# FrontierDevelopmentLab/2024-HL-SPI3S-SuNeRF

Hardware: AMD Instinct MI355X
Metric: ray-samples/sec (fwd+bwd, fused emission renderer) (higher is better)
Workload: dtype f32 (forward: every operand split into an fp16 head and an exact remainder, head products on the fp16 matrix cores + block-scaled fp8 products for the two cross terms; backward: fp16 MFMA, W^T as a single fp16 image (measured policy); fp32 accumulate and parameters)

## Files before the change

2024-hl-spi3s-sunerf_amd/csrc/bwd_pipe.hip:

```cpp
#include "grad_common.h"
#include <mutex>
#include <vector>

namespace {

constexpr int PD = 256, PKS = PD / 16, PNT = PD / 32, PT = 8;
constexpr int WG = 512;
constexpr int WG_PRE = 256;
constexpr int NBUF = 4;
constexpr int NBUF_H = 5;
#ifndef PIPE_DMA_ON_WEIGHT
#define PIPE_DMA_ON_WEIGHT 2
#endif
#ifndef PIPE_ZD
#define PIPE_ZD 2
#endif
#ifndef PIPE_RING
#define PIPE_RING 16
#endif
#ifndef PIPE_POLL_LAG
#define PIPE_POLL_LAG 2
#endif
constexpr int RING = PIPE_RING;
constexpr int SLOT = PKS * 1024;
constexpr int BUF_HID = 24 * 1024;
constexpr int BUF_IN = 16 * 1024;
constexpr int BUF_PRE = 19 * 1024;
constexpr unsigned SPIN_LIMIT = 50000000u;

constexpr unsigned ST_OK = 0, ST_START_TIMEOUT = 1, ST_PLACEMENT = 2, ST_WAIT_TIMEOUT = 3;

struct PipeArgs {
  const char* packedT;
  const char* act_stash;
  const char* dz_top;
  char* rings;
  unsigned* ctrl;
  float* partial;
  const float* g_raw;
  const unsigned* g_absmax_bits;
  float* partial_out;
  int64_t n_chunks_total;
  int S, n_chunks;
  int n_linear, d_out;
  int NP, NPX;
  int hi_only;
  int inject;
  unsigned* dbg;
};

__host__ __device__ inline size_t ctrl_counter_word(int n_links, int P, int link, int which) {
  return 64 + (((size_t)P * n_links + link) * 4 + which) * 32;
}
__host__ __device__ inline size_t ctrl_bytes(int NP, int n_links) { return (64 + (size_t)NP * n_links * 4 * 32) * 4; }

typedef __attribute__((address_space(1))) unsigned gu32;
__device__ __forceinline__ unsigned ld_agent(const unsigned* p) {
  return __hip_atomic_load((const gu32*)p, __ATOMIC_RELAXED, __HIP_MEMORY_SCOPE_AGENT);
}
__device__ __forceinline__ void st_agent(unsigned* p, unsigned v) {
  __hip_atomic_store((gu32*)p, v, __ATOMIC_RELAXED, __HIP_MEMORY_SCOPE_AGENT);
}

template <int POLICY>
__device__ __forceinline__ void dma_piece(const char* src_lane, unsigned lds_dst) {
  const unsigned d = __builtin_amdgcn_readfirstlane(lds_dst);
  if (POLICY == 1) asm volatile("s_mov_b32 m0, %1\n\ts_nop 0\n\tglobal_load_lds_dwordx4 %0, off nt" :: "v"(src_lane), "s"(d) : "memory");
  else if (POLICY == 2) asm volatile("s_mov_b32 m0, %1\n\ts_nop 0\n\tglobal_load_lds_dwordx4 %0, off sc1" :: "v"(src_lane), "s"(d) : "memory");
  else asm volatile("s_mov_b32 m0, %1\n\ts_nop 0\n\tglobal_load_lds_dwordx4 %0, off" :: "v"(src_lane), "s"(d) : "memory");
}
template <int POLICY>
__device__ __forceinline__ void dma_piece_s(const char* src_uniform, unsigned voff, unsigned lds_dst) {
  const unsigned d = __builtin_amdgcn_readfirstlane(lds_dst);
#ifndef PIPE_STREAM_BITS
#define PIPE_STREAM_BITS "nt"
#endif
  if (POLICY == 1) asm volatile("s_mov_b32 m0, %1\n\ts_nop 0\n\tglobal_load_lds_dwordx4 %0, %2 " PIPE_STREAM_BITS :: "v"(voff), "s"(d), "s"(src_uniform) : "memory");
  else if (POLICY == 2) asm volatile("s_mov_b32 m0, %1\n\ts_nop 0\n\tglobal_load_lds_dwordx4 %0, %2 sc1" :: "v"(voff), "s"(d), "s"(src_uniform) : "memory");
  else asm volatile("s_mov_b32 m0, %1\n\ts_nop 0\n\tglobal_load_lds_dwordx4 %0, %2" :: "v"(voff), "s"(d), "s"(src_uniform) : "memory");
}
__device__ __forceinline__ void dma_poll(const unsigned* src_lane, unsigned lds_dst) {
  const unsigned d = __builtin_amdgcn_readfirstlane(lds_dst);
  asm volatile("s_mov_b32 m0, %1\n\ts_nop 0\n\tglobal_load_lds_dword %0, off sc1" :: "v"(src_lane), "s"(d) : "memory");
}

__device__ __forceinline__ void store_tile(const f32x16& t, float* dst) {
  const Rsrc r = make_rsrc(dst, 16 * 64 * 4);
  const int lo4 = (int)(threadIdx.x & 63u) * 4;
#pragma unroll
  for (int g = 0; g < 16; ++g) {
    const float te = t[g];
    unsigned tv;
    asm volatile("v_accvgpr_read_b32 %0, %1" : "=v"(tv) : "a"(te));
    __builtin_amdgcn_raw_buffer_store_b32(tv, r, lo4, g * 256, 0);
    if ((g & 3) == 3) __builtin_amdgcn_sched_barrier(0);
  }
}

__device__ __forceinline__ void mfma_agpr(f32x16& acc, const half8& a, const half8& b) {
  asm volatile("v_mfma_f32_32x32x16_f16 %0, %1, %2, %0" : "+a"(acc) : "v"(a), "v"(b));
}
__device__ __forceinline__ void drain_matrix_pipe() { asm volatile("s_nop 15\n\ts_nop 15\n\ts_nop 15\n\ts_nop 15" ::: "memory"); }

#ifndef PIPE_KO_WREADS
#define PIPE_KO_WREADS 0
#endif
#if PIPE_KO_WREADS
#define TR_FIXED(R0, R1, R2, R3, OFF, var, base) asm volatile("" : "={v[" #R0 ":" #R3 "]}"(var) : "v"(base) : "memory")
#else
#define TR_FIXED(R0, R1, R2, R3, OFF, var, base)                                                                        \
  asm volatile("ds_read_b64_tr_b16 v[" #R0 ":" #R1 "], %1 offset:%2\n\tds_read_b64_tr_b16 v[" #R2 ":" #R3 "], %1 offset:%3" \
// ... 112 lines not shown
  const char* srcP0 = a.act_stash + SL.h_off(l - 1) + (size_t)(8 * j) * 1024;
  const int64_t safe = cbeg < a.n_chunks_total ? cbeg : a.n_chunks_total - 1;

  constexpr int ZD = TOP ? NBUF_H - 1 : PIPE_ZD;
  const char *nz = nullptr, *np = nullptr;
  unsigned zdst = 0, pdst = 0;
  bool zreal = false, preal = false;
  const char* const safe_p = srcP0 + (size_t)safe * act_chunk;
  const char* const safe_z = TOP ? a.dz_top + (size_t)safe * SLOT : ring_in;
  const char* run_p = srcP0 + (size_t)cbeg * act_chunk;
  const char* run_z = TOP ? a.dz_top + (size_t)cbeg * SLOT : ring_in;
  int run_slot = 0, run_zbuf = 0, run_pbuf = 0;
  auto next_p = [&](int nxt) __attribute__((always_inline)) {
    preal = nxt < n_my;
    pdst = lds0 + run_pbuf * BUF_HID + 16 * 1024;
    run_pbuf = run_pbuf + 1 == NBUF_H ? 0 : run_pbuf + 1;
    np = preal ? run_p : safe_p;
    run_p += act_chunk;
  };
  auto next_z = [&](int nxt) __attribute__((always_inline)) {
    if (nxt < 0) { zreal = false; nz = safe_z; return; }
    zreal = nxt < n_my;
    zdst = lds0 + run_zbuf * BUF_HID;
    run_zbuf = run_zbuf + 1 == NBUF_H ? 0 : run_zbuf + 1;
    nz = zreal ? run_z : safe_z;
    if (TOP) run_z += SLOT;
    else {
      run_slot = run_slot + 1 == RING ? 0 : run_slot + 1;
      run_z = run_slot == 0 ? ring_in : run_z + SLOT;
    }
  };
  auto piece_z = [&](int f) __attribute__((always_inline)) {
    const unsigned dst = zreal ? zdst + f * 1024 : lds_dummy;
    if (TOP) dma_piece_s<1>(nz + (size_t)f * 1024, voff, dst);
    else dma_piece_s<2>(nz + (size_t)f * 1024, voff, dst);
  };
  auto piece_p = [&](int f) __attribute__((always_inline)) { dma_piece_s<1>(np + (size_t)f * 1024, voff, preal ? pdst + f * 1024 : lds_dummy); };
  constexpr int NO = 2;
  constexpr int NP_D = PIPE_DMA_ON_WEIGHT == 0 ? 6 : PIPE_DMA_ON_WEIGHT == 1 ? 4 : 0;
  constexpr int NP_W = 6 - NP_D;
  constexpr int PER_D = NP_D + NO;
  auto min3 = [](int x, int y, int z) constexpr { return x < y ? (x < z ? x : z) : (y < z ? y : z); };
  constexpr int WAIT_LEFT = NP_D == 0 ? NO : min3((ZD - 1) * PER_D + (NP_D - 4) + NO, NP_D == 6 ? 2 * PER_D + NO : 63, 2 * PER_D);
  constexpr int DRAIN = (WAIT_LEFT + PER_D - 1) / PER_D + 1;
  auto w_wait = [min3](int per_w, bool gate_wave) constexpr {
    return min3(NP_W == 6 ? (ZD - 1) * per_w + 2 : 63, NP_W >= 2 ? 2 * per_w : 63, gate_wave ? PIPE_POLL_LAG * per_w - 2 : 63);
  };
  constexpr int W_WAIT_GATE = w_wait(NP_W + 2, true), W_WAIT_REST = w_wait(NP_W, false);

  static_assert(W_WAIT_GATE >= 0 && W_WAIT_GATE < 64 && WAIT_LEFT < 64, "vmcnt is a 6-bit counter");
  static_assert(ZD >= 1 && ZD <= NBUF_H - 1, "dZ fetch distance");

  if (wave < 4) {
#if defined(PIPE_PRIO) && PIPE_PRIO == 1
    __builtin_amdgcn_s_setprio(1);
#endif
#ifndef PIPE_PF
#define PIPE_PF 4
#endif
    constexpr int PF = PIPE_PF;
    const int U = 4 * j + wave;
    const int li = (a.n_linear - 2) - l;
    half8 wt_hi[PKS], wt_lo[HI_ONLY ? 1 : PKS];
    {
      const char* blk = a.packedT + (size_t)PNT * 1024 + ((size_t)li * PNT + U) * PKS * 2048 + lane * 16;
#pragma unroll
      for (int s = 0; s < PKS; ++s) {
        wt_hi[s] = *(const half8*)(blk + s * 2048);
        if constexpr (!HI_ONLY) wt_lo[s] = *(const half8*)(blk + s * 2048 + 1024);
      }
#pragma unroll
      for (int s = 0; s < PKS; ++s) {
        asm volatile("" : "+a"(wt_hi[s]));
        if constexpr (!HI_ONLY) asm volatile("" : "+a"(wt_lo[s]));
      }
    }
    char* scratch = a.rings + (size_t)a.NP * n_links * RING * SLOT + ((size_t)blockIdx.x * 4 + wave) * 2048;
    float cosn[16];
    v2f cosn2[8];
    typedef __attribute__((address_space(3))) v4u lds_v4u;
    typedef __attribute__((address_space(3))) half8 lds_half8;
    v4u dp[2];
    auto read_phases = [&](int b) __attribute__((always_inline)) {
      const unsigned at = lds0 + b * BUF_HID + (16 + 2 * wave) * 1024 + voff;
// ... 109 lines not shown
    if (PIPE_TRIM) {
#pragma unroll
      for (int q = 0; q < 8; ++q) { bs[2 * q] = bs2[q].x; bs[2 * q + 1] = bs2[q].y; }
    }
    store_bias_sums(bs, a.partial + ((size_t)(l - 1) * a.NP + P) * (PT * (PT + 1)) * 1024 + ((size_t)U * (PT + 1) + PT) * 1024);
    if (stamp && P == 0 && lane == 0) {
      unsigned long long* t = (unsigned long long*)(a.dbg + 256 * 8 * 4) + (((size_t)(blockIdx.x >> 3) * 8 + wave) * 8);
      for (int k = 0; k < 5; ++k) t[k] = tl[k];
    }
    if (stamp && wave == 1 && lane == 0) {
      unsigned* d = a.dbg + 256 * 8 + (size_t)blockIdx.x * 8;
      for (int k = 0; k < 6; ++k) d[k] = (unsigned)(ph[k] >> 4);
    }
    return;
  }

#if defined(PIPE_PRIO) && PIPE_PRIO == 2
  __builtin_amdgcn_s_setprio(1);
#endif
  const int v = wave - 4;
  const bool gatew = v == 0;
  const int rq = v >> 1, cq = v & 1;
  const int r0 = 4 * rq, c0 = 2 * cq;
  f32x16 acc[4][2];
  {
    half8 hz = {0, 0, 0, 0, 0, 0, 0, 0};
    asm volatile("s_nop 7" : "+v"(hz));
#pragma unroll
    for (int i = 0; i < 4; ++i) {
      asm volatile("v_mfma_f32_32x32x16_f16 %0, %1, %1, 0" : "=a"(acc[i][0]) : "v"(hz));
      asm volatile("v_mfma_f32_32x32x16_f16 %0, %1, %1, 0" : "=a"(acc[i][1]) : "v"(hz));
    }
  }
  unsigned* in_prod0 = a.ctrl + ctrl_counter_word(n_links, P, TOP ? 0 : l, 0);
  unsigned* in_prod1 = a.ctrl + ctrl_counter_word(n_links, P, TOP ? 0 : l, 1);
  unsigned* my_cons = a.ctrl + ctrl_counter_word(n_links, P, TOP ? 0 : l, 2 + j);
  unsigned* my_prod = a.ctrl + ctrl_counter_word(n_links, P, l - 1, j);
  unsigned* out_cons0 = a.ctrl + ctrl_counter_word(n_links, P, l - 1, 2 + (l == 1 ? j : 0));
  unsigned* out_cons1 = a.ctrl + ctrl_counter_word(n_links, P, l - 1, 2 + (l == 1 ? j : 1));
  const unsigned* poll_src = (lane & 3) == 0 ? in_prod0 : (lane & 3) == 1 ? in_prod1 : (lane & 3) == 2 ? out_cons0 : out_cons1;
  unsigned have_in = 0, have_out = 0;
  unsigned st_in[2] = {0, 0}, st_out[2] = {0, 0};
  const unsigned long long t_begin = __builtin_amdgcn_s_memrealtime();
  const unsigned laneoff = tr_lane_offset(lane);

  auto gate = [&](int itn) __attribute__((always_inline)) {
    const int nx = itn + ZD;
    const bool need_in = !TOP && nx >= 0 && nx < n_my && (int)(have_in - (unsigned)(nx + 1)) < 0;
    const bool need_out = itn >= RING && (int)(have_out - (unsigned)(itn - RING + 1)) < 0;
    if (need_in || need_out) {
      bool ok = true;
      if (lane == 0) {
        if (need_in) ok = spin_until(in_prod0, in_prod1, (unsigned)(nx + 1), status, have_in, st_in);
        if (ok && need_out) ok = spin_until(out_cons0, out_cons1, (unsigned)(itn - RING + 1), status, have_out, st_out);
        if (!ok) lds_st(lds_abort + (itn & 1) * 4, 1u);
      }
      have_in = __builtin_amdgcn_readfirstlane(have_in);
      have_out = __builtin_amdgcn_readfirstlane(have_out);
    }
  };
  if (gatew) {
    if (lane == 0) { lds_st(lds_abort, 0u); lds_st(lds_abort + 4, 0u); }
    gate(-(NBUF_H - 1));
  }

  bool aborted = false;
  unsigned long long tw = 0, tb = 0;
  unsigned long long t_wait = 0, t_bar = 0, tl[6] = {0, 0, 0, 0, 0, 0};
  const bool stamp = a.dbg != nullptr;
  int pslot = PIPE_POLL_LAG;
  auto top = [&](int it) __attribute__((always_inline)) {
    unsigned long long sa = 0, sb = 0;
    if (stamp) sa = __builtin_amdgcn_s_memtime();
    if (gatew) asm volatile("s_waitcnt vmcnt(%0)" :: "i"(W_WAIT_GATE) : "memory");
    else if (NP_W) asm volatile("s_waitcnt vmcnt(%0)" :: "i"(W_WAIT_REST) : "memory");
    if (stamp) sb = __builtin_amdgcn_s_memtime();
    barrier_mem();
    if (stamp) { t_wait = sb; t_bar = __builtin_amdgcn_s_memtime(); tw += sb - sa; tb += t_bar - sb; }
    const unsigned ab = lds_ld(lds_abort + (it & 1) * 4);
    if (gatew) {
      if (lane < 2) {
// ... 74 lines not shown
      ph[0] += s1 - s0; ph[1] += s2 - s1; ph[2] += s3 - s2;
      if (it == n_my / 2) { tl[0] = s0; tl[1] = t_wait; tl[2] = t_bar; tl[3] = s1; tl[4] = s2; tl[5] = s3; }
    }
    if (ab) { aborted = true; break; }
  }
  drain_matrix_pipe();
  if (stamp && (v == 0 || v == 1) && lane == 0) {
    unsigned* d = a.dbg + 256 * 8 * (2 + v) + (size_t)blockIdx.x * 8;
    for (int k = 0; k < 3; ++k) d[k] = (unsigned)(ph[k] >> 4);
    d[3] = (unsigned)(tw >> 4); d[4] = (unsigned)(tb >> 4);
  }
  if (stamp && P == 0 && lane == 0) {
    unsigned long long* t = (unsigned long long*)(a.dbg + 256 * 8 * 4) + (((size_t)(blockIdx.x >> 3) * 8 + wave) * 8);
    for (int k = 0; k < 6; ++k) t[k] = tl[k];
  }
  asm volatile("s_waitcnt vmcnt(0)" ::: "memory");
  barrier_mem();
  if (!aborted && gatew && lane < 2) st_agent(lane == 0 ? my_cons : my_prod, (unsigned)n_my);
  if (a.dbg && gatew && lane == 0) {
    unsigned* d = a.dbg + (size_t)blockIdx.x * 8;
    d[0] = (unsigned)(__builtin_amdgcn_s_memrealtime() - t_begin); d[1] = st_in[0]; d[2] = st_in[1]; d[3] = st_out[0]; d[4] = st_out[1];
    d[5] = (unsigned)n_my; d[6] = (unsigned)l; d[7] = (unsigned)P;
  }

  float* out = a.partial + ((size_t)l * a.NP + P) * (PT * (PT + 1)) * 1024;
#pragma unroll
  for (int i = 0; i < 4; ++i)
#pragma unroll
    for (int jj = 0; jj < 2; ++jj) {
      store_tile(acc[i][jj], out + ((size_t)(r0 + i) * (PT + 1) + (4 * j + c0 + jj)) * 1024);
    }
}

__device__ __forceinline__ void in_stage(const PipeArgs& a, char* smem, int P, int j, int64_t cbeg, int n_my) {
  constexpr int PW = 4;
  const int tid = threadIdx.x, lane = tid & 63;
  const int wave = __builtin_amdgcn_readfirstlane(tid >> 6);
  if (wave >= 4) {
    for (int it = -(NBUF - 1); it < n_my; ++it) {
      barrier_mem();
      if (lds_ld((unsigned)(uintptr_t)smem + NBUF * BUF_IN + 1024 + NBUF * 256 + (it & 1) * 4)) break;
    }
    barrier_mem();
    return;
  }
  const int n_act = a.n_linear - 1, n_links = n_act - 1;
  const StashLayout SL(PD, a.n_linear, true);
  const unsigned lds0 = (unsigned)(uintptr_t)smem;
  const unsigned lds_dummy = lds0 + NBUF * BUF_IN;
  const unsigned lds_poll = lds_dummy + 1024;
  const unsigned lds_abort = lds_poll + NBUF * 256;
  unsigned* status = a.ctrl;

  f32x16 acc[3];
#pragma unroll
  for (int c = 0; c < 3; ++c) acc[c] = (f32x16){0};

  const char* ring_in = a.rings + ((size_t)P * n_links + 0) * RING * SLOT;
  unsigned* in_prod = a.ctrl + ctrl_counter_word(n_links, P, 0, j);
  unsigned* my_cons = a.ctrl + ctrl_counter_word(n_links, P, 0, 2 + j);
  unsigned have_in = 0;
  unsigned st_in[2] = {0, 0};
  const unsigned long long t_begin = __builtin_amdgcn_s_memrealtime();
  const size_t act_chunk = SL.chunk_bytes();
  const unsigned laneoff = tr_lane_offset(lane);
  const int64_t safe = cbeg < a.n_chunks_total ? cbeg : a.n_chunks_total - 1;

  auto issue_chunk = [&](int c, int buf) __attribute__((always_inline)) {
    const bool real = c < n_my;
    const int64_t g = real ? cbeg + c : safe;
    const unsigned dst0 = lds0 + buf * BUF_IN;
    const char* z = ring_in + (size_t)((real ? c : 0) % RING) * SLOT + (size_t)(8 * j) * 1024 + lane * 16;
    const char* e = a.act_stash + (size_t)g * act_chunk + lane * 16;
#pragma unroll
    for (int k = 0; k < PW; ++k) {
      const int p = 4 * k + wave;
      if (k < 2) dma_piece<2>(z + (size_t)p * 1024, real ? dst0 + p * 1024 : lds_dummy);
      else {
        const bool use = real && p < 14;
        dma_piece<1>(e + (size_t)(p < 14 ? p - 8 : 0) * 1024, use ? dst0 + p * 1024 : lds_dummy);
      }
    }
  };

  bool aborted = false;
  for (int it = -(NBUF - 1); it < n_my; ++it) {
    const int buf = it & (NBUF - 1);
    const int nxt = it + NBUF - 1;
    if (wave == 0) asm volatile("s_waitcnt vmcnt(%0)" :: "i"(2 * (PW + 2)) : "memory");
    else asm volatile("s_waitcnt vmcnt(%0)" :: "i"(2 * PW) : "memory");
    if (wave == 0) {
      bool ok = true;
      if (it >= 0) {
        const unsigned p0 = lds_ld(lds_poll + buf * 256);
        if ((int)(p0 - have_in) > 0) have_in = p0;
      }
      if (lane == 0) {
        if (nxt < n_my && (int)(have_in - (unsigned)(nxt + 1)) < 0) ok = spin_until(in_prod, in_prod, (unsigned)(nxt + 1), status, have_in, st_in);
        lds_st(lds_abort + (it & 1) * 4, ok ? 0u : 1u);
      }
      have_in = __builtin_amdgcn_readfirstlane(have_in);
    }
    barrier_mem();
    if (lds_ld(lds_abort + (it & 1) * 4)) { aborted = true; break; }
    if (wave == 0) {
      if (lane == 0) st_agent(my_cons, (unsigned)(it + 1 > 0 ? it + 1 : 0));
      dma_poll(in_prod, lds_poll + (nxt & (NBUF - 1)) * 256);
    }
    issue_chunk(nxt, nxt & (NBUF - 1));
    if (it < 0) continue;
#if defined(PIPE_ABL_IN_STAGE) && PIPE_ABL_IN_STAGE
    continue;
#endif
    const unsigned bufA = lds0 + buf * BUF_IN + laneoff, bufB = bufA + 8 * 1024;
#pragma unroll
    for (int ks = 0; ks < 2; ++ks) {
      half4 alo, ahi, blo[3], bhi[3];
// ... 44 lines not shown
    const unsigned old = __hip_atomic_fetch_or((gu32*)(a.ctrl + 8 + x), mine, __ATOMIC_RELAXED, __HIP_MEMORY_SCOPE_AGENT);
    asm volatile("s_waitcnt vmcnt(0)" ::: "memory");
    (void)old;
    __hip_atomic_fetch_add((gu32*)(a.ctrl + 1), 1u, __ATOMIC_RELAXED, __HIP_MEMORY_SCOPE_AGENT);
    bool ok = true;
    const unsigned long long t0 = __builtin_amdgcn_s_memrealtime();
    while (ld_agent(a.ctrl + 1) < gridDim.x) {
      if (ld_agent(status) != ST_OK) { ok = false; break; }
      if (__builtin_amdgcn_s_memrealtime() - t0 > SPIN_LIMIT) { st_agent(status, ST_START_TIMEOUT); ok = false; break; }
      __builtin_amdgcn_s_sleep(8);
    }
    if (ok) {
      const unsigned m = ld_agent(a.ctrl + 8 + x);
      if (__builtin_popcount(m) != 1) { st_agent(status, ST_PLACEMENT); ok = false; }
    }
    lds_st(start_ok, ok ? 1u : 0u);
  }
  __syncthreads();
  const bool ok = lds_ld(start_ok) != 0;

  const int q = i / per_pipe;
  if (q >= a.NPX) return;
  const int r = i % per_pipe, si = r >> 1, j = r & 1;
  const int l = n_act - 1 - si;
  const int P = q * 8 + x;
  const int64_t per = (a.n_chunks_total + a.NP - 1) / a.NP;
  const int64_t cbeg = (int64_t)P * per;
  int64_t cend = cbeg + per;
  if (cend > a.n_chunks_total) cend = a.n_chunks_total;
  const int n_my = (ok && cend > cbeg) ? (int)(cend - cbeg) : 0;
  if (l == 0) in_stage(a, smem, P, j, cbeg, n_my);
  else if (l == n_act - 1) hidden_stage<HI_ONLY, true>(a, smem, P, l, j, cbeg, n_my);
  else hidden_stage<HI_ONLY, false>(a, smem, P, l, j, cbeg, n_my);
}

__global__ __launch_bounds__(WG_PRE, 1) void bwd_prologue_kernel(PipeArgs a) {
  constexpr int PW = 4, NO = 4;
  extern __shared__ __attribute__((aligned(16))) char smem[];
  const int tid = threadIdx.x, lane = tid & 63;
  const int wave = __builtin_amdgcn_readfirstlane(tid >> 6);
  const int n = lane & 31, h = lane >> 5;
  const int n_act = a.n_linear - 1;
  const StashLayout SL(PD, a.n_linear, true);
  const unsigned lds0 = (unsigned)(uintptr_t)smem;
  const unsigned lds_dummy = lds0 + NBUF * BUF_PRE;
  const float gscale = sunerf_gscale(*a.g_absmax_bits);

  const int64_t per = (a.n_chunks_total + gridDim.x - 1) / gridDim.x;
  const int64_t cbeg = (int64_t)blockIdx.x * per;
  int64_t cend = cbeg + per;
  if (cend > a.n_chunks_total) cend = a.n_chunks_total;
  const int n_my = cend > cbeg ? (int)(cend - cbeg) : 0;
  const int64_t safe = cbeg < a.n_chunks_total ? cbeg : a.n_chunks_total - 1;

  half8 aT[2];
#pragma unroll
  for (int t = 0; t < 2; ++t) aT[t] = *(const half8*)(a.packedT + (size_t)(2 * wave + t) * 1024 + lane * 16);

  f32x16 acc[2] = {(f32x16){0}, (f32x16){0}};
  float bs[2][16];
#pragma unroll
  for (int g = 0; g < 16; ++g) { bs[0][g] = 0.f; bs[1][g] = 0.f; }
  float gsum0 = 0.f, gsum1 = 0.f;
  const size_t act_chunk = SL.chunk_bytes();
  const char* srcP0 = a.act_stash + SL.h_off(n_act - 1) + (size_t)(4 * wave) * 1024 + lane * 16;
  const unsigned laneoff = tr_lane_offset(lane);
  char* scratch = a.rings + (size_t)a.NP * (n_act - 1) * RING * SLOT + ((size_t)blockIdx.x * 4 + wave) * 2048;
  typedef __attribute__((address_space(3))) v4u lds_v4u;
  typedef __attribute__((address_space(3))) half8 lds_half8;

  auto issue_chunk = [&](int c, int buf) __attribute__((always_inline)) {
    const bool real = c < n_my;
    const int64_t g = real ? cbeg + c : safe;
    const unsigned dst0 = lds0 + buf * BUF_PRE;
    if (wave == 0) {
      const int64_t ray = g / a.n_chunks;
      const int c32 = (int)(g % a.n_chunks) * 32;
      if (c32 + (lane >> 1) < a.S) dma_poll((const unsigned*)(a.g_raw + ((size_t)ray * a.S + c32) * 2 + lane), real ? dst0 + 18 * 1024 : lds_dummy);
    }
#pragma unroll
    for (int k = 0; k < PW; ++k)
      dma_piece<1>(srcP0 + (size_t)g * act_chunk + (size_t)k * 1024, real ? dst0 + (4 * wave + k) * 1024 : lds_dummy);
  };

  for (int it = -(NBUF - 1); it < n_my; ++it) {
    const int buf = it & (NBUF - 1);
    const int nxt = it + NBUF - 1;
    if (wave == 0) asm volatile("s_waitcnt vmcnt(%0)" :: "i"(NO + 2 * (PW + NO + 1)) : "memory");
    else asm volatile("s_waitcnt vmcnt(%0)" :: "i"(NO + 2 * (PW + NO)) : "memory");
    half8 dzo = {0, 0, 0, 0, 0, 0, 0, 0};
    float cs[2][16];
    if (it >= 0) {
#pragma unroll
      for (int f = 0; f < 4; ++f) {
        const unsigned at = lds0 + buf * BUF_PRE + (4 * wave + f) * 1024 + lane * 16;
        const v4u p = *(const lds_v4u*)(uintptr_t)at;
        float sn[8];
        decode_phases(p, sn, cs[f >> 1] + 8 * (f & 1));
        *(lds_half8*)(uintptr_t)at = to_half8(sn);
      }
      const int64_t chunk = cbeg + it;
      const int c = (int)(chunk % a.n_chunks);
      const int i = 32 * c + n;
      if (h == 0 && i < a.S) {
        const f32x2 g = *(const f32x2*)(smem + (size_t)buf * BUF_PRE + 18 * 1024 + n * 8);
        const float g0 = g[0] * gscale, g1 = a.d_out > 1 ? g[1] * gscale : 0.f;
        dzo[0] = (_Float16)g0;
        dzo[1] = (_Float16)g1;
        gsum0 += g0;
        gsum1 += g1;
      }
      if (wave == 0) *(half8*)(smem + (size_t)buf * BUF_PRE + 16 * 1024 + lane * 16) = dzo;
      else if (wave == 1) *(half8*)(smem + (size_t)buf * BUF_PRE + 17 * 1024 + lane * 16) = (half8){0, 0, 0, 0, 0, 0, 0, 0};
    }
    barrier_mem();
    issue_chunk(nxt, nxt & (NBUF - 1));
    if (it < 0) {
      const Rsrc sc = make_rsrc(scratch, 2048);
      const half8 zero = {0, 0, 0, 0, 0, 0, 0, 0};
#pragma unroll
      for (int k = 0; k < NO; ++k) buf_store(zero, sc, (k & 1) * 1024);
      continue;
    }
    const Rsrc ro = make_rsrc(a.dz_top + (size_t)(cbeg + it) * SLOT, SLOT);
#pragma unroll
    for (int t = 0; t < 2; ++t) {
      const int U = 2 * wave + t;
      f32x16 d = {0};
      d = __builtin_amdgcn_mfma_f32_32x32x16_f16(aT[t], dzo, d, 0, 0, 0);
      half8 d0, d1;
      dz_tile(d, cs[t], cs[t] + 8, d0, d1, bs[t]);
      buf_store(d0, ro, (2 * U) * 1024);
      buf_store(d1, ro, (2 * U + 1) * 1024);
    }
    const unsigned bufH = lds0 + buf * BUF_PRE + laneoff, bufA = bufH + 16 * 1024;
#pragma unroll
    for (int ks = 0; ks < 2; ++ks) {
      half4 alo, ahi, blo[2], bhi[2];
      tr_issue(bufA + ks * 256, alo, ahi);
#pragma unroll
      for (int t = 0; t < 2; ++t) tr_issue(bufH + (2 * (2 * wave + t)) * 1024 + ks * 256, blo[t], bhi[t]);
      asm volatile("s_waitcnt lgkmcnt(0)" ::: "memory");
      asm volatile("" : "+v"(alo), "+v"(ahi));
#pragma unroll
      for (int t = 0; t < 2; ++t) asm volatile("" : "+v"(blo[t]), "+v"(bhi[t]));
      const half8 af = join(alo, ahi);
#pragma unroll
      for (int t = 0; t < 2; ++t) acc[t] = __builtin_amdgcn_mfma_f32_32x32x16_f16(af, join(blo[t], bhi[t]), acc[t], 0, 0, 0);
    }
  }
  asm volatile("s_waitcnt vmcnt(0)" ::: "memory");
  float* out = a.partial_out + (size_t)blockIdx.x * (PT + 2) * 1024;
#pragma unroll
  for (int t = 0; t < 2; ++t) {
    store_tile(acc[t], out + (size_t)(2 * wave + t) * 1024);
    store_bias_sums(bs[t], out + (size_t)(PT + 1) * 1024 + (2 * wave + t) * 32);
  }
  if (wave == 0) {
#pragma unroll
    for (int d = 16; d >= 1; d >>= 1) { gsum0 += __shfl_xor(gsum0, d, 32); gsum1 += __shfl_xor(gsum1, d, 32); }
    if (lane < 32) out[(size_t)PT * 1024 + lane] = lane == 0 ? gsum0 : (lane == 1 ? gsum1 : 0.f);
  }
}

struct PipeLayout {
  int n_act, n_links, NPX, NP, grid;
  size_t sticky, dbg, ctrl, rings, dz_top, partial, partial_out, total;
  PipeLayout(int64_t n_chunks_total, int n_linear, int cus) {
    n_act = n_linear - 1;
    n_links = n_act - 1;
    grid = cus;
    NPX = (cus / 8) / (2 * n_act);
    NP = 8 * NPX;
    auto up = [](size_t v) { return (v + 255) / 256 * 256; };
    size_t off = 0;
    sticky = off; off += SUNERF_PIPE_WS_DEBUG;
    dbg = off; off += up((size_t)cus * 64 * sizeof(unsigned));
    ctrl = off; off += up(ctrl_bytes(NP, n_links));
    rings = off; off += up((size_t)NP * n_links * RING * SLOT + (size_t)cus * 4 * 2048);
    dz_top = off; off += up((size_t)(n_chunks_total > 0 ? n_chunks_total : 1) * SLOT);
    partial = off; off += up((size_t)n_act * NP * PT * (PT + 1) * 1024 * sizeof(float));
    partial_out = off; off += up((size_t)cus * (PT + 2) * 1024 * sizeof(float));
    total = off;
  }
};
static_assert(SUNERF_PIPE_WS_STICKY == 0 && SUNERF_PIPE_WS_DEBUG == 256, "fixed offsets of the workspace header");

struct TimedLaunch { hipEvent_t e0, e1; };
std::mutex g_timed_mutex;
std::vector<TimedLaunch> g_timed;

bool pipe_supported(int d_filter, int n_linear, int d_out, int cus) {
  return d_filter == PD && n_linear >= 3 && n_linear <= SUNERF_MAX_LAYERS && d_out >= 1 && d_out <= 2 && cus == 256 &&
         2 * (n_linear - 1) <= cus / 8;
}

int device_cus() {
  int dev = 0, cus = 0;
  (void)hipGetDevice(&dev);
  (void)hipDeviceGetAttribute(&cus, hipDeviceAttributeMultiprocessorCount, dev);
  return cus;
}

}

extern "C" size_t sunerf_bwd_pipe_workspace_bytes(int64_t n_rays, int n_samples, int d_filter, int n_linear) {
  const int cus = device_cus();
  if (n_rays < 0 || n_samples < 2 || !pipe_supported(d_filter, n_linear, 1, cus)) return 0;
  const int64_t n_chunks = (n_samples + 31) / 32;
  return PipeLayout(n_rays * n_chunks, n_linear, cus).total;
}

extern "C" int sunerf_mlp_backward_pipe(int d_filter, int n_linear, int d_out, const void* packedT, const void* act_stash,
                                        const float* g_raw, const void* g_absmax, int64_t n_rays, int n_samples,
                                        void* workspace, size_t workspace_bytes, float* const* grad_weights_host,
                                        float* const* grad_biases_host, int accumulate, int flags, void* stream) {
  if (!grad_weights_host || !grad_biases_host) return SUNERF_E_BADARG;
  if (n_rays <= 0 || n_samples < 2) return SUNERF_E_BADARG;
  if (!packedT || !act_stash || !g_raw || !g_absmax || !workspace) return SUNERF_E_BADARG;
  const int cus = device_cus();
  if (!pipe_supported(d_filter, n_linear, d_out, cus)) return SUNERF_E_UNSUPPORTED;
  hipStream_t st = (hipStream_t)stream;
  const int n_chunks = (n_samples + 31) / 32;
  const PipeLayout L(n_rays * n_chunks, n_linear, cus);
  if (workspace_bytes < L.total) return SUNERF_E_WORKSPACE;
  char* ws = (char*)workspace;
  PipeArgs a;
  a.packedT = (const char*)packedT; a.act_stash = (const char*)act_stash; a.dz_top = ws + L.dz_top; a.rings = ws + L.rings;
  a.ctrl = (unsigned*)(ws + L.ctrl); a.partial = (float*)(ws + L.partial); a.g_raw = g_raw;
  a.g_absmax_bits = (const unsigned*)g_absmax; a.partial_out = (float*)(ws + L.partial_out);
  a.n_chunks_total = n_rays * n_chunks; a.S = n_samples; a.n_chunks = n_chunks; a.n_linear = n_linear; a.d_out = d_out;
  a.NP = L.NP; a.NPX = L.NPX; a.hi_only = flags & 1; a.inject = (flags >> 8) & 1;
  a.dbg = (flags & 2) ? (unsigned*)(ws + L.dbg) : nullptr;
  hipError_t e;
  if ((e = hipMemsetAsync(ws + L.ctrl, 0, L.rings - L.ctrl, st)) != hipSuccess) return (int)e;
  const size_t lds_pre = (size_t)NBUF * BUF_PRE + 1024;
  const size_t lds_pipe = (size_t)NBUF_H * BUF_HID + 1024 + NBUF_H * 256 + 64;
  if ((e = hipFuncSetAttribute((const void*)bwd_prologue_kernel, hipFuncAttributeMaxDynamicSharedMemorySize, (int)lds_pre)) != hipSuccess) return (int)e;
  if ((e = hipFuncSetAttribute((const void*)bwd_pipe_kernel<false>, hipFuncAttributeMaxDynamicSharedMemorySize, (int)lds_pipe)) != hipSuccess) return (int)e;
  if ((e = hipFuncSetAttribute((const void*)bwd_pipe_kernel<true>, hipFuncAttributeMaxDynamicSharedMemorySize, (int)lds_pipe)) != hipSuccess) return (int)e;
  TimedLaunch tl = {nullptr, nullptr};
  if (flags & 0x80) {
    if ((e = hipEventCreate(&tl.e0)) != hipSuccess) return (int)e;
    if ((e = hipEventCreate(&tl.e1)) != hipSuccess) { (void)hipEventDestroy(tl.e0); return (int)e; }
  }
  SUNERF_CLEAR_ERROR();
  hipLaunchKernelGGL(bwd_prologue_kernel, dim3((unsigned)cus), dim3(WG_PRE), lds_pre, st, a);
  SUNERF_CHECK_LAUNCH();
  if (tl.e0) (void)hipEventRecord(tl.e0, st);
  if (a.hi_only) hipLaunchKernelGGL(bwd_pipe_kernel<true>, dim3((unsigned)cus), dim3(WG), lds_pipe, st, a);
  else hipLaunchKernelGGL(bwd_pipe_kernel<false>, dim3((unsigned)cus), dim3(WG), lds_pipe, st, a);
  if (tl.e0) {
    (void)hipEventRecord(tl.e1, st);
    std::lock_guard<std::mutex> lock(g_timed_mutex);
    g_timed.push_back(tl);
  }
  SUNERF_CHECK_LAUNCH();
  ReduceArgs r;
  const size_t slot = (size_t)PT * (PT + 1) * 1024;
  for (int i = 0; i < n_linear; ++i) {
    if (!grad_weights_host[i] || !grad_biases_host[i]) return SUNERF_E_BADARG;
    r.gW[i] = grad_weights_host[i];
    r.gb[i] = grad_biases_host[i];
    if (i < n_linear - 1) {
      r.partial[i] = a.partial + (size_t)i * L.NP * slot;
      r.split[i] = L.NP;
      r.slot[i] = slot;
    } else {
      r.partial[i] = a.partial_out;
      r.split[i] = cus;
      r.slot[i] = (size_t)(PT + 2) * 1024;
    }
    if (i < n_linear - 2) {
      r.bias[i] = r.partial[i] + (size_t)PT * 1024;
      r.bias_split[i] = L.NP;
      r.bias_slot[i] = slot;
      r.bias_tr[i] = (size_t)(PT + 1) * 1024;
    } else {
      r.bias[i] = a.partial_out + (size_t)(i == n_linear - 1 ? PT : PT + 1) * 1024;
      r.bias_split[i] = cus;
      r.bias_slot[i] = (size_t)(PT + 2) * 1024;
      r.bias_tr[i] = 32;
    }
  }
  r.g_absmax_bits = (const unsigned*)g_absmax; r.n_linear = n_linear; r.D = d_filter; r.d_out = d_out; r.accumulate = accumulate;
  r.sumsq = (const float*)((const char*)packedT + sunerf_packed_mlp_t_bytes(d_filter, n_linear) - SUNERF_MAX_LAYERS * sizeof(float));
  r.status = a.ctrl;
  r.sticky = (unsigned*)(ws + L.sticky);
  hipLaunchKernelGGL(reduce_grads_kernel, dim3(PT * (PT + 1) * 1024 / 256, n_linear), dim3(256), 0, st, r);
  SUNERF_CHECK_LAUNCH();
  return 0;
}

extern "C" int sunerf_bwd_pipe_kernel_time(double* total_ms, int* launches) {
  std::vector<TimedLaunch> mine;
  {
    std::lock_guard<std::mutex> lock(g_timed_mutex);
    mine.swap(g_timed);
  }
  double sum = 0.0;
  int n = 0, rc = 0;
  for (const TimedLaunch& t : mine) {
    float ms = 0.f;
    hipError_t e = hipEventSynchronize(t.e1);
    if (e == hipSuccess) e = hipEventElapsedTime(&ms, t.e0, t.e1);
    if (e == hipSuccess) { sum += ms; ++n; } else rc = (int)e;
    (void)hipEventDestroy(t.e0);
    (void)hipEventDestroy(t.e1);
  }
  if (total_ms) *total_ms = sum;
  if (launches) *launches = n;
  return rc;
}
// ... 1 lines not shown
```

Measured before the change: 199.9 million.

## Fold output-layer prologue into pipelined backward kernel as a producer stage

Removes the separate bwd_prologue_kernel, which computed the output-layer dZ and its weight gradient before the pipe kernel started. That work now runs in the previously idle waves 4-7 of the in-layer stage, and a new control link lets the top hidden stage wait on that producer's progress counter instead of assuming dZ is complete. This removes one launch and the serial prologue phase, overlapping it with the hidden-layer pipeline. In exchange it adds a lead and flow-control dependency that could stall the pipeline, changes the partial_out split to NP, and uses nontemporal stores for dz_top.

```diff
diff --git a/2024-hl-spi3s-sunerf_amd/csrc/bwd_pipe.hip b/2024-hl-spi3s-sunerf_amd/csrc/bwd_pipe.hip
--- a/2024-hl-spi3s-sunerf_amd/csrc/bwd_pipe.hip
+++ b/2024-hl-spi3s-sunerf_amd/csrc/bwd_pipe.hip
@@ -6,8 +6,9 @@
 
 constexpr int PD = 256, PKS = PD / 16, PNT = PD / 32, PT = 8;
 constexpr int WG = 512;
-constexpr int WG_PRE = 256;
 constexpr int NBUF = 4;
+constexpr int NBUF_P = 4;
+constexpr int OUT_GROUP = 16;
 constexpr int NBUF_H = 5;
 #ifndef PIPE_DMA_ON_WEIGHT
 #define PIPE_DMA_ON_WEIGHT 2
@@ -20,12 +21,22 @@
 #endif
 #ifndef PIPE_POLL_LAG
 #define PIPE_POLL_LAG 2
+#endif
+#ifndef PIPE_TOP_STORE_NT
+#define PIPE_TOP_STORE_NT 1
+#endif
+#ifndef PIPE_TOP_READ_NT
+#define PIPE_TOP_READ_NT 0
+#endif
+#ifndef PIPE_LEAD
+#define PIPE_LEAD 8
 #endif
 constexpr int RING = PIPE_RING;
 constexpr int SLOT = PKS * 1024;
 constexpr int BUF_HID = 24 * 1024;
 constexpr int BUF_IN = 16 * 1024;
-constexpr int BUF_PRE = 19 * 1024;
+constexpr int BUF_OUT = 9 * 1024;
+constexpr int LDS_OUT = 68 * 1024;
 constexpr unsigned SPIN_LIMIT = 50000000u;
 
 constexpr unsigned ST_OK = 0, ST_START_TIMEOUT = 1, ST_PLACEMENT = 2, ST_WAIT_TIMEOUT = 3;
@@ -33,7 +44,7 @@
 struct PipeArgs {
   const char* packedT;
   const char* act_stash;
-  const char* dz_top;
+  char* dz_top;
   char* rings;
   unsigned* ctrl;
   float* partial;
@@ -50,9 +61,9 @@
 };
 
 __host__ __device__ inline size_t ctrl_counter_word(int n_links, int P, int link, int which) {
-  return 64 + (((size_t)P * n_links + link) * 4 + which) * 32;
-}
-__host__ __device__ inline size_t ctrl_bytes(int NP, int n_links) { return (64 + (size_t)NP * n_links * 4 * 32) * 4; }
+  return 64 + (((size_t)P * (n_links + 1) + link) * 4 + which) * 32;
+}
+__host__ __device__ inline size_t ctrl_bytes(int NP, int n_links) { return (64 + (size_t)NP * (n_links + 1) * 4 * 32) * 4; }
 
 typedef __attribute__((address_space(1))) unsigned gu32;
 __device__ __forceinline__ unsigned ld_agent(const unsigned* p) {
@@ -77,6 +88,7 @@
 #endif
   if (POLICY == 1) asm volatile("s_mov_b32 m0, %1\n\ts_nop 0\n\tglobal_load_lds_dwordx4 %0, %2 " PIPE_STREAM_BITS :: "v"(voff), "s"(d), "s"(src_uniform) : "memory");
   else if (POLICY == 2) asm volatile("s_mov_b32 m0, %1\n\ts_nop 0\n\tglobal_load_lds_dwordx4 %0, %2 sc1" :: "v"(voff), "s"(d), "s"(src_uniform) : "memory");
+  else if (POLICY == 3) asm volatile("s_mov_b32 m0, %1\n\ts_nop 0\n\tglobal_load_lds_dwordx4 %0, %2 sc1 nt" :: "v"(voff), "s"(d), "s"(src_uniform) : "memory");
   else asm volatile("s_mov_b32 m0, %1\n\ts_nop 0\n\tglobal_load_lds_dwordx4 %0, %2" :: "v"(voff), "s"(d), "s"(src_uniform) : "memory");
 }
 __device__ __forceinline__ void dma_poll(const unsigned* src_lane, unsigned lds_dst) {
@@ -255,7 +267,7 @@
   };
   auto piece_z = [&](int f) __attribute__((always_inline)) {
     const unsigned dst = zreal ? zdst + f * 1024 : lds_dummy;
-    if (TOP) dma_piece_s<1>(nz + (size_t)f * 1024, voff, dst);
+    if (TOP && PIPE_TOP_READ_NT) dma_piece_s<3>(nz + (size_t)f * 1024, voff, dst);
     else dma_piece_s<2>(nz + (size_t)f * 1024, voff, dst);
   };
   auto piece_p = [&](int f) __attribute__((always_inline)) { dma_piece_s<1>(np + (size_t)f * 1024, voff, preal ? pdst + f * 1024 : lds_dummy); };
@@ -273,6 +285,7 @@
 
   static_assert(W_WAIT_GATE >= 0 && W_WAIT_GATE < 64 && WAIT_LEFT < 64, "vmcnt is a 6-bit counter");
   static_assert(ZD >= 1 && ZD <= NBUF_H - 1, "dZ fetch distance");
+  static_assert(ZD + DRAIN <= PIPE_LEAD, "out_producer: the lead per layer must cover what a stage asks of the stage above it");
 
   if (wave < 4) {
 #if defined(PIPE_PRIO) && PIPE_PRIO == 1
@@ -448,9 +461,10 @@
       asm volatile("v_mfma_f32_32x32x16_f16 %0, %1, %1, 0" : "=a"(acc[i][1]) : "v"(hz));
     }
   }
-  unsigned* in_prod0 = a.ctrl + ctrl_counter_word(n_links, P, TOP ? 0 : l, 0);
-  unsigned* in_prod1 = a.ctrl + ctrl_counter_word(n_links, P, TOP ? 0 : l, 1);
-  unsigned* my_cons = a.ctrl + ctrl_counter_word(n_links, P, TOP ? 0 : l, 2 + j);
+  const int in_link = TOP ? n_links : l;
+  unsigned* in_prod0 = a.ctrl + ctrl_counter_word(n_links, P, in_link, 0);
+  unsigned* in_prod1 = a.ctrl + ctrl_counter_word(n_links, P, in_link, 1);
+  unsigned* my_cons = a.ctrl + ctrl_counter_word(n_links, P, in_link, 2 + j);
   unsigned* my_prod = a.ctrl + ctrl_counter_word(n_links, P, l - 1, j);
   unsigned* out_cons0 = a.ctrl + ctrl_counter_word(n_links, P, l - 1, 2 + (l == 1 ? j : 0));
   unsigned* out_cons1 = a.ctrl + ctrl_counter_word(n_links, P, l - 1, 2 + (l == 1 ? j : 1));
@@ -462,7 +476,7 @@
 
   auto gate = [&](int itn) __attribute__((always_inline)) {
     const int nx = itn + ZD;
-    const bool need_in = !TOP && nx >= 0 && nx < n_my && (int)(have_in - (unsigned)(nx + 1)) < 0;
+    const bool need_in = nx >= 0 && nx < n_my && (int)(have_in - (unsigned)(nx + 1)) < 0;
     const bool need_out = itn >= RING && (int)(have_out - (unsigned)(itn - RING + 1)) < 0;
     if (need_in || need_out) {
       bool ok = true;
@@ -603,16 +617,151 @@
     }
 }
 
+__device__ __forceinline__ int out_lead(int n_act, int n_my) {
+  const int lead = NBUF + NBUF_P + PIPE_LEAD * n_act, few = n_my + NBUF + NBUF_P + 1;
+  return few < lead ? few : lead;
+}
+
+__device__ __forceinline__ void out_producer(const PipeArgs& a, char* smem, int P, int j, int64_t cbeg, int n_my) {
+  const int tid = threadIdx.x, lane = tid & 63;
+  const int v = __builtin_amdgcn_readfirstlane(tid >> 6) - 4;
+  const int n = lane & 31, h = lane >> 5;
+  const int U = 4 * j + v;
+  const int n_act = a.n_linear - 1, n_links = n_act - 1;
+  const int lead = out_lead(n_act, n_my);
+  const StashLayout SL(PD, a.n_linear, true);
+  const unsigned lds0 = (unsigned)(uintptr_t)smem;
+  const unsigned lds_dummy = lds0 + NBUF * BUF_IN;
+  const unsigned lds_abort = lds_dummy + 1024 + NBUF * 256;
+  const unsigned lds_stage = lds0 + LDS_OUT;
+  const unsigned lds_op = lds_stage + NBUF_P * BUF_OUT + v * 2048;
+  const float gscale = sunerf_gscale(*a.g_absmax_bits);
+  const int64_t safe = cbeg < a.n_chunks_total ? cbeg : a.n_chunks_total - 1;
+  typedef __attribute__((address_space(3))) v4u lds_v4u;
+  typedef __attribute__((address_space(3))) half8 lds_half8;
+
+  const half8 aT = *(const half8*)(a.packedT + (size_t)U * 1024 + lane * 16);
+  *(lds_half8*)(uintptr_t)(lds_op + 1024 + lane * 16) = (half8){0, 0, 0, 0, 0, 0, 0, 0};
+
+  unsigned* my_prod = a.ctrl + ctrl_counter_word(n_links, P, n_links, j);
+  char* scratch = a.rings + (size_t)a.NP * n_links * RING * SLOT + ((size_t)blockIdx.x * 4 + v) * 2048;
+  const size_t act_chunk = SL.chunk_bytes();
+  const char* srcP = a.act_stash + SL.h_off(n_act - 1) + (size_t)(2 * U) * 1024 + lane * 16;
+  const char* run_p = srcP + (size_t)safe * act_chunk;
+  int64_t f_ray = safe / a.n_chunks;
+  int f_cr = (int)(safe % a.n_chunks);
+  const int64_t s_ray = f_ray;
+  const int s_cr = f_cr;
+  int k_cr = f_cr;
+
+  f32x16 acc = {0}, tot = {0};
+  float bs[16];
+#pragma unroll
+  for (int g = 0; g < 16; ++g) bs[g] = 0.f;
+  float gsum0 = 0.f, gsum1 = 0.f;
+  const unsigned laneoff = tr_lane_offset(lane);
+  bool aborted = false;
+
+  for (int it = -(lead + NBUF_P - 1); it < n_my; ++it) {
+    const int c = it + lead, f = c + NBUF_P - 1;
+    if (v == 0) asm volatile("s_waitcnt vmcnt(%0)" :: "i"(2 + (NBUF_P - 2) * 6) : "memory");
+    else asm volatile("s_waitcnt vmcnt(%0)" :: "i"(2 + (NBUF_P - 2) * 5) : "memory");
+    barrier_mem();
+    if (it >= -(NBUF - 1) && lds_ld(lds_abort + (it & 1) * 4)) { aborted = true; break; }
+    if (v == 0 && lane == 0) {
+      int pv = it - NBUF_P + lead + 1;
+      pv = pv < 0 ? 0 : pv > n_my ? n_my : pv;
+      st_agent(my_prod, (unsigned)pv);
+    }
+    {
+      const bool real = f >= 0 && f < n_my;
+      const unsigned dst = lds_stage + (f & (NBUF_P - 1)) * BUF_OUT;
+      const int64_t ray = real ? f_ray : s_ray;
+      const int c32 = (real ? f_cr : s_cr) * 32;
+      if (c32 + (lane >> 1) < a.S) dma_poll((const unsigned*)(a.g_raw + ((size_t)ray * a.S + c32) * 2 + lane), real ? dst + 8 * 1024 + v * 256 : lds_dummy);
+      const char* src = real ? run_p : srcP + (size_t)safe * act_chunk;
+      dma_piece<1>(src, real ? dst + (2 * v) * 1024 : lds_dummy);
+      dma_piece<1>(src + 1024, real ? dst + (2 * v + 1) * 1024 : lds_dummy);
+      if (real) {
+        run_p += act_chunk;
+        if (++f_cr == a.n_chunks) { f_cr = 0; ++f_ray; }
+      }
+    }
+    const bool make = c >= 0 && c < n_my;
+    half8 d0 = {0, 0, 0, 0, 0, 0, 0, 0}, d1 = d0;
+    const unsigned cb = lds_stage + (c & (NBUF_P - 1)) * BUF_OUT;
+    if (make) {
+      float cs[16];
+#pragma unroll
+      for (int fr = 0; fr < 2; ++fr) {
+        const unsigned at = cb + (2 * v + fr) * 1024 + lane * 16;
+        const v4u p = *(const lds_v4u*)(uintptr_t)at;
+        float sn[8];
+        decode_phases(p, sn, cs + 8 * fr);
+        *(lds_half8*)(uintptr_t)at = to_half8(sn);
+      }
+      half8 dzo = {0, 0, 0, 0, 0, 0, 0, 0};
+      const int i = 32 * k_cr + n;
+      if (h == 0 && i < a.S) {
+        const f32x2 g = *(const f32x2*)(smem + (size_t)(cb - lds0) + 8 * 1024 + v * 256 + n * 8);
+        const float g0 = g[0] * gscale, g1 = a.d_out > 1 ? g[1] * gscale : 0.f;
+        dzo[0] = (_Float16)g0;
+        dzo[1] = (_Float16)g1;
+        gsum0 += g0;
+        gsum1 += g1;
+      }
+      *(lds_half8*)(uintptr_t)(lds_op + lane * 16) = dzo;
+      f32x16 d = {0};
+      d = __builtin_amdgcn_mfma_f32_32x32x16_f16(aT, dzo, d, 0, 0, 0);
+      dz_tile(d, cs, cs + 8, d0, d1, bs);
+      if (++k_cr == a.n_chunks) k_cr = 0;
+    }
+    {
+      const Rsrc ro = make ? make_rsrc(a.dz_top + (size_t)(cbeg + c) * SLOT, SLOT) : make_rsrc(scratch, 2048);
+      if (PIPE_TOP_STORE_NT) {
+        buf_store_nt(d0, ro, make ? (2 * U) * 1024 : 0);
+        buf_store_nt(d1, ro, make ? (2 * U + 1) * 1024 : 1024);
+      } else {
+        buf_store(d0, ro, make ? (2 * U) * 1024 : 0);
+        buf_store(d1, ro, make ? (2 * U + 1) * 1024 : 1024);
+      }
+    }
+    if (make) {
+#pragma unroll
+      for (int ks = 0; ks < 2; ++ks) {
+        half4 alo, ahi, blo, bhi;
+        tr_issue(lds_op + laneoff + ks * 256, alo, ahi);
+        tr_issue(cb + (2 * v) * 1024 + laneoff + ks * 256, blo, bhi);
+        asm volatile("s_waitcnt lgkmcnt(0)" ::: "memory");
+        asm volatile("" : "+v"(alo), "+v"(ahi), "+v"(blo), "+v"(bhi));
+        acc = __builtin_amdgcn_mfma_f32_32x32x16_f16(join(alo, ahi), join(blo, bhi), acc, 0, 0, 0);
+      }
+      if ((c & (OUT_GROUP - 1)) == OUT_GROUP - 1) {
+        tot += acc;
+        acc = (f32x16){0};
+      }
+    }
+  }
+  tot += acc;
+  asm volatile("s_waitcnt vmcnt(0)" ::: "memory");
+  barrier_mem();
+  if (!aborted && v == 0 && lane == 0) st_agent(my_prod, (unsigned)n_my);
+  float* out = a.partial_out + (size_t)P * (PT + 2) * 1024;
+  store_tile(tot, out + (size_t)U * 1024);
+  store_bias_sums(bs, out + (size_t)(PT + 1) * 1024 + U * 32);
+  if (j == 0 && v == 0) {
+#pragma unroll
+    for (int d = 16; d >= 1; d >>= 1) { gsum0 += __shfl_xor(gsum0, d, 32); gsum1 += __shfl_xor(gsum1, d, 32); }
+    if (lane < 32) out[(size_t)PT * 1024 + lane] = lane == 0 ? gsum0 : (lane == 1 ? gsum1 : 0.f);
+  }
+}
+
 __device__ __forceinline__ void in_stage(const PipeArgs& a, char* smem, int P, int j, int64_t cbeg, int n_my) {
   constexpr int PW = 4;
   const int tid = threadIdx.x, lane = tid & 63;
   const int wave = __builtin_amdgcn_readfirstlane(tid >> 6);
   if (wave >= 4) {
-    for (int it = -(NBUF - 1); it < n_my; ++it) {
-      barrier_mem();
-      if (lds_ld((unsigned)(uintptr_t)smem + NBUF * BUF_IN + 1024 + NBUF * 256 + (it & 1) * 4)) break;
-    }
-    barrier_mem();
+    out_producer(a, smem, P, j, cbeg, n_my);
     return;
   }
   const int n_act = a.n_linear - 1, n_links = n_act - 1;
@@ -654,6 +803,7 @@
     }
   };
 
+  for (int it = -(out_lead(n_act, n_my) + NBUF_P - 1); it < -(NBUF - 1); ++it) barrier_mem();
   bool aborted = false;
   for (int it = -(NBUF - 1); it < n_my; ++it) {
     const int buf = it & (NBUF - 1);
@@ -764,135 +914,6 @@
   if (l == 0) in_stage(a, smem, P, j, cbeg, n_my);
   else if (l == n_act - 1) hidden_stage<HI_ONLY, true>(a, smem, P, l, j, cbeg, n_my);
   else hidden_stage<HI_ONLY, false>(a, smem, P, l, j, cbeg, n_my);
-}
-
-__global__ __launch_bounds__(WG_PRE, 1) void bwd_prologue_kernel(PipeArgs a) {
-  constexpr int PW = 4, NO = 4;
-  extern __shared__ __attribute__((aligned(16))) char smem[];
-  const int tid = threadIdx.x, lane = tid & 63;
-  const int wave = __builtin_amdgcn_readfirstlane(tid >> 6);
-  const int n = lane & 31, h = lane >> 5;
-  const int n_act = a.n_linear - 1;
-  const StashLayout SL(PD, a.n_linear, true);
-  const unsigned lds0 = (unsigned)(uintptr_t)smem;
-  const unsigned lds_dummy = lds0 + NBUF * BUF_PRE;
-  const float gscale = sunerf_gscale(*a.g_absmax_bits);
-
-  const int64_t per = (a.n_chunks_total + gridDim.x - 1) / gridDim.x;
-  const int64_t cbeg = (int64_t)blockIdx.x * per;
-  int64_t cend = cbeg + per;
-  if (cend > a.n_chunks_total) cend = a.n_chunks_total;
-  const int n_my = cend > cbeg ? (int)(cend - cbeg) : 0;
-  const int64_t safe = cbeg < a.n_chunks_total ? cbeg : a.n_chunks_total - 1;
-
-  half8 aT[2];
-#pragma unroll
-  for (int t = 0; t < 2; ++t) aT[t] = *(const half8*)(a.packedT + (size_t)(2 * wave + t) * 1024 + lane * 16);
-
-  f32x16 acc[2] = {(f32x16){0}, (f32x16){0}};
-  float bs[2][16];
-#pragma unroll
-  for (int g = 0; g < 16; ++g) { bs[0][g] = 0.f; bs[1][g] = 0.f; }
-  float gsum0 = 0.f, gsum1 = 0.f;
-  const size_t act_chunk = SL.chunk_bytes();
-  const char* srcP0 = a.act_stash + SL.h_off(n_act - 1) + (size_t)(4 * wave) * 1024 + lane * 16;
-  const unsigned laneoff = tr_lane_offset(lane);
-  char* scratch = a.rings + (size_t)a.NP * (n_act - 1) * RING * SLOT + ((size_t)blockIdx.x * 4 + wave) * 2048;
-  typedef __attribute__((address_space(3))) v4u lds_v4u;
-  typedef __attribute__((address_space(3))) half8 lds_half8;
-
-  auto issue_chunk = [&](int c, int buf) __attribute__((always_inline)) {
-    const bool real = c < n_my;
-    const int64_t g = real ? cbeg + c : safe;
-    const unsigned dst0 = lds0 + buf * BUF_PRE;
-    if (wave == 0) {
-      const int64_t ray = g / a.n_chunks;
-      const int c32 = (int)(g % a.n_chunks) * 32;
-      if (c32 + (lane >> 1) < a.S) dma_poll((const unsigned*)(a.g_raw + ((size_t)ray * a.S + c32) * 2 + lane), real ? dst0 + 18 * 1024 : lds_dummy);
-    }
-#pragma unroll
-    for (int k = 0; k < PW; ++k)
-      dma_piece<1>(srcP0 + (size_t)g * act_chunk + (size_t)k * 1024, real ? dst0 + (4 * wave + k) * 1024 : lds_dummy);
-  };
-
-  for (int it = -(NBUF - 1); it < n_my; ++it) {
-    const int buf = it & (NBUF - 1);
-    const int nxt = it + NBUF - 1;
-    if (wave == 0) asm volatile("s_waitcnt vmcnt(%0)" :: "i"(NO + 2 * (PW + NO + 1)) : "memory");
-    else asm volatile("s_waitcnt vmcnt(%0)" :: "i"(NO + 2 * (PW + NO)) : "memory");
-    half8 dzo = {0, 0, 0, 0, 0, 0, 0, 0};
-    float cs[2][16];
-    if (it >= 0) {
-#pragma unroll
-      for (int f = 0; f < 4; ++f) {
-        const unsigned at = lds0 + buf * BUF_PRE + (4 * wave + f) * 1024 + lane * 16;
-        const v4u p = *(const lds_v4u*)(uintptr_t)at;
-        float sn[8];
-        decode_phases(p, sn, cs[f >> 1] + 8 * (f & 1));
-        *(lds_half8*)(uintptr_t)at = to_half8(sn);
-      }
-      const int64_t chunk = cbeg + it;
-      const int c = (int)(chunk % a.n_chunks);
-      const int i = 32 * c + n;
-      if (h == 0 && i < a.S) {
-        const f32x2 g = *(const f32x2*)(smem + (size_t)buf * BUF_PRE + 18 * 1024 + n * 8);
-        const float g0 = g[0] * gscale, g1 = a.d_out > 1 ? g[1] * gscale : 0.f;
-        dzo[0] = (_Float16)g0;
-        dzo[1] = (_Float16)g1;
-        gsum0 += g0;
-        gsum1 += g1;
-      }
-      if (wave == 0) *(half8*)(smem + (size_t)buf * BUF_PRE + 16 * 1024 + lane * 16) = dzo;
-      else if (wave == 1) *(half8*)(smem + (size_t)buf * BUF_PRE + 17 * 1024 + lane * 16) = (half8){0, 0, 0, 0, 0, 0, 0, 0};
-    }
-    barrier_mem();
-    issue_chunk(nxt, nxt & (NBUF - 1));
-    if (it < 0) {
-      const Rsrc sc = make_rsrc(scratch, 2048);
-      const half8 zero = {0, 0, 0, 0, 0, 0, 0, 0};
-#pragma unroll
-      for (int k = 0; k < NO; ++k) buf_store(zero, sc, (k & 1) * 1024);
-      continue;
-    }
-    const Rsrc ro = make_rsrc(a.dz_top + (size_t)(cbeg + it) * SLOT, SLOT);
-#pragma unroll
-    for (int t = 0; t < 2; ++t) {
-      const int U = 2 * wave + t;
-      f32x16 d = {0};
-      d = __builtin_amdgcn_mfma_f32_32x32x16_f16(aT[t], dzo, d, 0, 0, 0);
-      half8 d0, d1;
-      dz_tile(d, cs[t], cs[t] + 8, d0, d1, bs[t]);
-      buf_store(d0, ro, (2 * U) * 1024);
-      buf_store(d1, ro, (2 * U + 1) * 1024);
-    }
-    const unsigned bufH = lds0 + buf * BUF_PRE + laneoff, bufA = bufH + 16 * 1024;
-#pragma unroll
-    for (int ks = 0; ks < 2; ++ks) {
-      half4 alo, ahi, blo[2], bhi[2];
-      tr_issue(bufA + ks * 256, alo, ahi);
-#pragma unroll
-      for (int t = 0; t < 2; ++t) tr_issue(bufH + (2 * (2 * wave + t)) * 1024 + ks * 256, blo[t], bhi[t]);
-      asm volatile("s_waitcnt lgkmcnt(0)" ::: "memory");
-      asm volatile("" : "+v"(alo), "+v"(ahi));
-#pragma unroll
-      for (int t = 0; t < 2; ++t) asm volatile("" : "+v"(blo[t]), "+v"(bhi[t]));
-      const half8 af = join(alo, ahi);
-#pragma unroll
-      for (int t = 0; t < 2; ++t) acc[t] = __builtin_amdgcn_mfma_f32_32x32x16_f16(af, join(blo[t], bhi[t]), acc[t], 0, 0, 0);
-    }
-  }
-  asm volatile("s_waitcnt vmcnt(0)" ::: "memory");
-  float* out = a.partial_out + (size_t)blockIdx.x * (PT + 2) * 1024;
-#pragma unroll
-  for (int t = 0; t < 2; ++t) {
-    store_tile(acc[t], out + (size_t)(2 * wave + t) * 1024);
-    store_bias_sums(bs[t], out + (size_t)(PT + 1) * 1024 + (2 * wave + t) * 32);
-  }
-  if (wave == 0) {
-#pragma unroll
-    for (int d = 16; d >= 1; d >>= 1) { gsum0 += __shfl_xor(gsum0, d, 32); gsum1 += __shfl_xor(gsum1, d, 32); }
-    if (lane < 32) out[(size_t)PT * 1024 + lane] = lane == 0 ? gsum0 : (lane == 1 ? gsum1 : 0.f);
-  }
 }
 
 struct PipeLayout {
@@ -912,7 +933,7 @@
     rings = off; off += up((size_t)NP * n_links * RING * SLOT + (size_t)cus * 4 * 2048);
     dz_top = off; off += up((size_t)(n_chunks_total > 0 ? n_chunks_total : 1) * SLOT);
     partial = off; off += up((size_t)n_act * NP * PT * (PT + 1) * 1024 * sizeof(float));
-    partial_out = off; off += up((size_t)cus * (PT + 2) * 1024 * sizeof(float));
+    partial_out = off; off += up((size_t)NP * (PT + 2) * 1024 * sizeof(float));
     total = off;
   }
 };
@@ -966,9 +987,12 @@
   a.dbg = (flags & 2) ? (unsigned*)(ws + L.dbg) : nullptr;
   hipError_t e;
   if ((e = hipMemsetAsync(ws + L.ctrl, 0, L.rings - L.ctrl, st)) != hipSuccess) return (int)e;
-  const size_t lds_pre = (size_t)NBUF * BUF_PRE + 1024;
   const size_t lds_pipe = (size_t)NBUF_H * BUF_HID + 1024 + NBUF_H * 256 + 64;
-  if ((e = hipFuncSetAttribute((const void*)bwd_prologue_kernel, hipFuncAttributeMaxDynamicSharedMemorySize, (int)lds_pre)) != hipSuccess) return (int)e;
+  static_assert(LDS_OUT >= NBUF * BUF_IN + 1024 + NBUF * 256 + 8, "out-layer producer staging behind the in-layer stage's");
+  static_assert(LDS_OUT + NBUF_P * BUF_OUT + 4 * 2048 <= NBUF_H * BUF_HID, "out-layer producer staging in front of the start-up word");
+  static_assert((NBUF_P & (NBUF_P - 1)) == 0 && NBUF_P >= 2, "NBUF_P: a power of two (buffer = chunk & (NBUF_P - 1))");
+  for (int i = 0; i < n_linear; ++i)
+    if (!grad_weights_host[i] || !grad_biases_host[i]) return SUNERF_E_BADARG;
   if ((e = hipFuncSetAttribute((const void*)bwd_pipe_kernel<false>, hipFuncAttributeMaxDynamicSharedMemorySize, (int)lds_pipe)) != hipSuccess) return (int)e;
   if ((e = hipFuncSetAttribute((const void*)bwd_pipe_kernel<true>, hipFuncAttributeMaxDynamicSharedMemorySize, (int)lds_pipe)) != hipSuccess) return (int)e;
   TimedLaunch tl = {nullptr, nullptr};
@@ -977,21 +1001,21 @@
     if ((e = hipEventCreate(&tl.e1)) != hipSuccess) { (void)hipEventDestroy(tl.e0); return (int)e; }
   }
   SUNERF_CLEAR_ERROR();
-  hipLaunchKernelGGL(bwd_prologue_kernel, dim3((unsigned)cus), dim3(WG_PRE), lds_pre, st, a);
-  SUNERF_CHECK_LAUNCH();
   if (tl.e0) (void)hipEventRecord(tl.e0, st);
   if (a.hi_only) hipLaunchKernelGGL(bwd_pipe_kernel<true>, dim3((unsigned)cus), dim3(WG), lds_pipe, st, a);
   else hipLaunchKernelGGL(bwd_pipe_kernel<false>, dim3((unsigned)cus), dim3(WG), lds_pipe, st, a);
+  if (tl.e0) (void)hipEventRecord(tl.e1, st);
+  if ((e = hipGetLastError()) != hipSuccess) {
+    if (tl.e0) { (void)hipEventDestroy(tl.e0); (void)hipEventDestroy(tl.e1); }
+    return (int)e;
+  }
   if (tl.e0) {
-    (void)hipEventRecord(tl.e1, st);
     std::lock_guard<std::mutex> lock(g_timed_mutex);
     g_timed.push_back(tl);
   }
-  SUNERF_CHECK_LAUNCH();
   ReduceArgs r;
   const size_t slot = (size_t)PT * (PT + 1) * 1024;
   for (int i = 0; i < n_linear; ++i) {
-    if (!grad_weights_host[i] || !grad_biases_host[i]) return SUNERF_E_BADARG;
     r.gW[i] = grad_weights_host[i];
     r.gb[i] = grad_biases_host[i];
     if (i < n_linear - 1) {
@@ -1000,7 +1024,7 @@
       r.slot[i] = slot;
     } else {
       r.partial[i] = a.partial_out;
-      r.split[i] = cus;
+      r.split[i] = L.NP;
       r.slot[i] = (size_t)(PT + 2) * 1024;
     }
     if (i < n_linear - 2) {
@@ -1010,7 +1034,7 @@
       r.bias_tr[i] = (size_t)(PT + 1) * 1024;
     } else {
       r.bias[i] = a.partial_out + (size_t)(i == n_linear - 1 ? PT : PT + 1) * 1024;
-      r.bias_split[i] = cus;
+      r.bias_split[i] = L.NP;
       r.bias_slot[i] = (size_t)(PT + 2) * 1024;
       r.bias_tr[i] = 32;
     }
```

Measured after the change: 201.5 million (median of 6 runs). Within noise of the previous version (+0.8%).
